# kalj/dealii-cuda

Hardware: AMD Instinct MI355X
Metric: DoFs/s on 1305x Laplace vmult (bmop), p=4 3D uniform (higher is better)
Workload: dtype f64; 1 GPU; bmop: DEGREE_FE=4, DIMENSION=3, MATRIX_FREE_UNIFORM_MESH, hyper_cube(-1,1), 54^3 cells, 10218313 DoFs, 1 z-slab(s); cells_per_dir=54, n_dofs=10218313, n_cells=157464, parallelism=slab1, dof_numbering=caller's (lexicographic), finite=True, clock_ramp_steps=2000

## Files before the change

### dealii-cuda_amd/csrc/mfgpu_kernels_p.hip

```cpp
#include <hip/hip_runtime.h>

#include "mfgpu_cell.h"
#include "mfgpu_kernels.h"
#include "mfgpu_planes.h"

namespace mfgpu {

#define MFGPU_PIN_VMEM() __builtin_amdgcn_sched_barrier(0x380)

template <int n, typename T, bool ADD, bool HN, bool SH = false, bool MASS = false>
__global__ void __launch_bounds__(64) __attribute__((amdgpu_waves_per_eu(1, 1)))
apply_planes3(const ApplyArgs<T> A, const TablesEO<T, n> tab) {
  constexpr int n2 = n * n;
  constexpr int CW = p_cells_per_wave(n);
  constexpr int NT = CW * n;
  constexpr int KGU = p_kgu(n);
  constexpr int JI = p_ji(n);
  constexpr int HS = KGU - JI;
  constexpr int SA = p_cell_stride(n);
  constexpr int NIW = (n2 + 1) / 2;
  extern __shared__ __attribute__((aligned(16))) unsigned char smem_raw[];
  constexpr int PRIV = HN ? p_priv_max(n) : 0;
  double *ua = reinterpret_cast<double *>(smem_raw);
  T *Aw = reinterpret_cast<T *>(ua + KGU * 64 + PRIV + (HN ? n2 : 0));
  T *Bw = Aw + (CW + 1) * SA;
  double *Wl = ua + KGU * 64 + PRIV;

  const int lane = threadIdx.x;
  if (HN) {
    if (lane < n2) Wl[lane] = (double)A.hn_weights[lane];
  }
  const int lc = lane / n, k = lane - lc * n;
  const bool lane_on = lane < NT;
  const int tk = lane_on ? lane : NT - 1;

  uint32_t b, bstride, bend;
  {
    const uint32_t nbt = A.batch_end - A.batch0 - A.hole_len, G = gridDim.x;
    if (G >= 8 && nbt >= G) {
      const uint32_t xcd = blockIdx.x & 7u, slot = blockIdx.x >> 3;
      const uint32_t q = G >> 3, rem = G & 7u;
      const uint32_t wlo = xcd * q + (xcd < rem ? xcd : rem);
      const uint32_t w = q + (xcd < rem ? 1u : 0u);
      b = A.batch0 + (uint32_t)((uint64_t)nbt * wlo / G) + slot;
      bend = A.batch0 + (uint32_t)((uint64_t)nbt * (wlo + w) / G);
      bstride = w;
    } else {
      b = A.batch0 + blockIdx.x;
      bend = A.batch_end - A.hole_len;
      bstride = G;
    }
  }
  if (b >= bend) return;
  const uint32_t hole0 = A.hole0, hole_len = A.hole_len;
  auto next_of = [&](uint32_t x) {
    const uint32_t l = (x >= hole0 ? x - hole_len : x) + bstride;
    return l < bend ? (l >= hole0 ? l + hole_len : l) : x;
  };
  if (b >= hole0) b += hole_len;
  static_assert(kernel_exists(PlaneKernel::planes3, n, number_type_of<T>, HN, SH, MASS), "no such instantiation");
  struct Meta {
    uint32_t base, drec, irec;
  };
  auto meta_request = [&](uint32_t bb) -> uint32_t {
    return A.shtab[(size_t)bb * kShBatchWords + (lane & (kShBatchWords - 1))];
  };
  auto meta_of = [&](uint32_t v) -> Meta {
    return Meta{(uint32_t)__builtin_amdgcn_readlane((int)v, 0), (uint32_t)__builtin_amdgcn_readlane((int)v, 1),
                (uint32_t)__builtin_amdgcn_readlane((int)v, 2)};
  };

  auto load_dofs = [&](uint32_t rec, uint32_t (&g)[KGU]) {
    const uint32_t *p = A.bdofsp + (size_t)rec * (KGU * 64) + lane;
#pragma unroll
    for (int j = 0; j < KGU; ++j) g[j] = SH ? p[j * 64] : nt_load(p + j * 64);
  };
  auto src_at = [&](uint32_t base, uint32_t g) -> T {
    const T *const sp = SH ? A.src + base : A.src;
    return *reinterpret_cast<const T *>(reinterpret_cast<const char *>(sp) + (uint32_t)(g * (uint32_t)sizeof(T)));
  };
  auto dst_at = [&](uint32_t base, uint32_t g) -> T * {
    T *const dp = SH ? A.dst + base : A.dst;
    return reinterpret_cast<T *>(reinterpret_cast<char *>(dp) + (uint32_t)(g * (uint32_t)sizeof(T)));
  };
  auto load_ix = [&](uint32_t rec, uint32_t (&ix)[NIW]) {
    const uint32_t *p = A.idxp + (size_t)rec * (NIW * NT) + tk;
#pragma unroll
    for (int w = 0; w < NIW; ++w) ix[w] = SH ? p[w * NT] : nt_load(p + w * NT);
  };
  auto stage_src = [&](const uint32_t (&g)[KGU], const T (&sv)[KGU]) {
#pragma unroll
    for (int j = 0; j < KGU; ++j) {
      double v = (double)sv[j];
      if (j >= JI) {
        const unsigned long long keep = (unsigned long long)(long long)~((int)g[j] >> 31);
        v = __longlong_as_double((long long)((unsigned long long)__double_as_longlong(v) & keep));
      }
      ua[lane + j * 64] = v;
    }
  };
  auto ixb = [&](const uint32_t (&ix)[NIW], int i) -> uint32_t {
    return (i & 1) ? (ix[i >> 1] >> 16) : (ix[i >> 1] & 0xffffu);
  };
  auto scatter_slot = [&](int j, uint32_t bb, uint32_t base, uint32_t g, T r, T oldv) {
    if (j < JI) {
      *dst_at(base, g) = ADD ? oldv + r : r;
    } else {
      T *const hp = A.halo + (size_t)bb * (HS * 64) + lane;
      hp[(j - JI) * 64] = r;
    }
  };

  uint32_t b1 = next_of(b), b2 = next_of(b1);
  uint32_t Gp[KGU], Gc[KGU], Gn[KGU], Gnn[KGU];
  uint32_t IXc[NIW], IXn[NIW];
  constexpr int CR = PRIV / 64, HROWS = HN ? p_hn_rows(n) : 1;
  uint32_t Hc[HROWS], Hn[HROWS];
  auto load_hn = [&](uint32_t bb, uint32_t (&H)[HROWS]) {
    const uint32_t slot = A.hn_slot[bb];
    if (slot != 0xffffffffu) {
      const uint32_t *p = A.hnrec + (size_t)slot * (HROWS * 64) + lane;
#pragma unroll
      for (int w = 0; w < HROWS; ++w) H[w] = nt_load(p + w * 64);
    } else {
#pragma unroll
      for (int w = 0; w < HROWS; ++w) H[w] = 0u;
    }
  };
  T Cc[n2];
  T Mm[MASS ? n2 : 1];
  T SVn[KGU], R[KGU], old[KGU];
  Meta Mp{0u, 0u, 0u}, Mc = Mp, M1 = Mp, M2 = Mp;
  uint32_t Mv = 0u;
  if (SH) {
    Mc = meta_of(meta_request(b));
    M1 = meta_of(meta_request(b1));
    M2 = meta_of(meta_request(b2));
    Mp = Mc;
  }
  load_dofs(SH ? Mc.drec : b, Gc);
  load_dofs(SH ? M1.drec : b1, Gn);
  load_ix(SH ? Mc.irec : b, IXc);
  if (HN) load_hn(b, Hc);
  constexpr uint32_t kDummyIx = 8u * (uint32_t)(KGU * 64 - 1) * 0x10001u;
#pragma unroll
  for (int w = 0; w < NIW; ++w) IXc[w] = lane_on ? IXc[w] : kDummyIx;
  {
    const T *p = A.coefp + (size_t)b * (n2 * NT) + tk;
#pragma unroll
    for (int r = 0; r < n2; ++r) Cc[r] = nt_load(p + r * NT);
  }
  if (MASS) {
    const T *p = A.massp + (size_t)b * (n2 * NT) + tk;
#pragma unroll
    for (int r = 0; r < n2; ++r) Mm[r] = nt_load(p + r * NT);
  }
#pragma unroll
  for (int j = 0; j < KGU; ++j) {
    SVn[j] = src_at(Mc.base, Gc[j]);
    Gp[j] = Gc[j];
    R[j] = T(0);
    old[j] = T(0);
  }
  stage_src(Gc, SVn);
  WaveSync::sync();

  const int pxy = lc * SA + n2 * k;
  const int pyz = lc * SA + k;
  uint32_t bp = b;

  while (true) {
    const bool has_next = b1 != b;
    constexpr int kH2 = HN ? HROWS - 2 : 0, kH1 = HN ? HROWS - 1 : 0;
    const uint32_t hn_ncopy = HN ? (uint32_t)__builtin_amdgcn_readfirstlane(Hc[kH2] & 0xffffu) : 0u;
    auto hn_count = [&](int dir) -> uint32_t {
      const uint32_t w = dir == 0 ? Hc[kH2] >> 16 : dir == 1 ? Hc[kH1] & 0xffffu : Hc[kH1] >> 16;
      return (uint32_t)__builtin_amdgcn_readfirstlane(w);
    };
    auto hn_pass = [&](int dir, bool transposed, const double (&Wr)[n2]) {
      const uint32_t count = hn_count(dir);
#pragma unroll
      for (int r = 0; r < kHnOpRounds; ++r) {
        if ((uint32_t)(r * 64) >= count) break;
        const bool on = (uint32_t)(r * 64 + lane) < count;
        const uint32_t *ww = &Hc[CR + (dir * kHnOpRounds + r) * 3];
        double v[n], o[n];
        uint32_t pos[n];
#pragma unroll
        for (int t = 0; t < n; ++t) {
          pos[t] = on ? (ww[t >> 1] >> (16 * (t & 1))) & 0xffffu : (uint32_t)(KGU * 64 + PRIV - 1);
          v[t] = ua[pos[t]];
        }
#pragma unroll
        for (int i = 0; i < n; ++i) {
          double acc = 0.0;
#pragma unroll
          for (int k2 = 0; k2 < n; ++k2) acc = fma(transposed ? Wr[k2 * n + i] : Wr[i * n + k2], v[k2], acc);
          o[i] = acc;
        }
        if (on) {
#pragma unroll
          for (int i = 0; i < n; ++i) ua[pos[i]] = o[i];
        }
      }
    };
    if (HN && hn_ncopy) {
      double Wr[n2];
#pragma unroll
      for (int i = 0; i < n2; ++i) Wr[i] = Wl[i];
      double cv[CR > 0 ? CR : 1];
#pragma unroll
      for (int r = 0; r < CR; ++r) cv[r] = (uint32_t)(r * 64 + lane) < hn_ncopy ? ua[Hc[r] & 0xffffu] : 0.0;
#pragma unroll
      for (int r = 0; r < CR; ++r)
        if ((uint32_t)(r * 64 + lane) < hn_ncopy) ua[Hc[r] >> 16] = cv[r];
      WaveSync::sync();
      hn_pass(0, false, Wr);
      WaveSync::sync();
      hn_pass(1, false, Wr);
      WaveSync::sync();
      hn_pass(2, false, Wr);
      WaveSync::sync();
    }
    STAMP(0);
    RSTAMP(8);
    WGSTAMP(10);
    load_dofs(SH ? M2.drec : b2, Gnn);
    load_ix(SH ? M1.irec : b1, IXn);
    if (SH) Mv = meta_request(next_of(b2));
    if (HN) load_hn(b1, Hn);
    if (ADD) {
#pragma unroll
      for (int j = 0; j < JI; ++j) old[j] = *dst_at(Mp.base, Gp[j]);
    }
    STAMP(1);
    auto hookA = [&](int) {};
    auto hookB = [&](int s) {
      MFGPU_PIN_VMEM();
#pragma unroll
      for (int j = (KGU * s) / (5 * n); j < (KGU * (s + 1)) / (5 * n); ++j)
        scatter_slot(j, bp, Mp.base, Gp[j], R[j], old[j]);
#pragma unroll
      for (int j = (KGU * s) / (5 * n); j < (KGU * (s + 1)) / (5 * n); ++j)
        SVn[j] = src_at(M1.base, Gn[j]);
      MFGPU_PIN_VMEM();
    };
    const T *const cnext = A.coefp + (size_t)b1 * (n2 * NT) + tk;
    const T *const mnext = MASS ? A.massp + (size_t)b1 * (n2 * NT) + tk : nullptr;
    auto hookC = [&](int s) {
      MFGPU_PIN_VMEM();
#pragma unroll
      for (int r = (n2 * s) / (2 * n); r < (n2 * (s + 1)) / (2 * n); ++r)
        Cc[r] = nt_load(cnext + r * NT);
      if (MASS) {
#pragma unroll
        for (int r = (n2 * s) / (2 * n); r < (n2 * (s + 1)) / (2 * n); ++r)
          Mm[r] = nt_load(mnext + r * NT);
      }
      MFGPU_PIN_VMEM();
    };

    {
      T u[n2];
#pragma unroll
      for (int x = 0; x < n; ++x)
#pragma unroll
        for (int y = 0; y < n; ++y)
          u[x + n * y] = (T) * reinterpret_cast<const double *>(reinterpret_cast<const char *>(ua) + ixb(IXc, x + n * y));
#pragma unroll
      for (int x = 0; x < n; ++x) {
        T in[n], out[n];
        get_line<n, 1>(u, x, in);
        eo_apply<n, 0>(tab, in, out);
        set_line<n, 1>(u, x, out);
        hookA(x);
      }
#pragma unroll
      for (int y = 0; y < n; ++y) {
        T in[n], a[n], bb[n];
        get_line<n, 0>(u, y, in);
        eo_apply<n, 0>(tab, in, a);
        eo_apply<n, 2>(tab, a, bb);
#pragma unroll
        for (int x = 0; x < n; ++x) {
          Aw[pxy + x + n * y] = a[x];
          Bw[pxy + x + n * y] = bb[x];
        }
        hookA(n + y);
      }
    }
    WaveSync::sync();
    STAMP(2);
#pragma unroll
    for (int j = 0; j < KGU + PRIV / 64; ++j) ua[lane + j * 64] = 0.0;

    {
      T nx[n];
#pragma unroll
      for (int z = 0; z < n; ++z) nx[z] = Bw[pyz + n2 * z];
#pragma unroll
      for (int y = 0; y < n; ++y) {
        T in[n], g[n], o[n];
#pragma unroll
        for (int z = 0; z < n; ++z) in[z] = nx[z];
#pragma unroll
        for (int z = 0; z < n; ++z) nx[z] = y + 1 < n ? Bw[pyz + n * (y + 1) + n2 * z] : Aw[pyz + n2 * z];
        eo_apply<n, 0>(tab, in, g);
#pragma unroll
        for (int z = 0; z < n; ++z) g[z] *= Cc[y + n * z];
        eo_apply<n, 1>(tab, g, o);
#pragma unroll
        for (int z = 0; z < n; ++z) Bw[pyz + n * y + n2 * z] = o[z];
        hookB(y);
      }
      T v[n2], r[n2];
#pragma unroll
      for (int y = 0; y < n; ++y) {
        T in[n], o[n];
#pragma unroll
        for (int z = 0; z < n; ++z) in[z] = nx[z];
        if (y + 1 < n) {
#pragma unroll
          for (int z = 0; z < n; ++z) nx[z] = Aw[pyz + n * (y + 1) + n2 * z];
        }
        eo_apply<n, 0>(tab, in, o);
        set_line<n, 1>(v, y, o);
        hookB(n + y);
      }
#pragma unroll
      for (int y = 0; y < n; ++y) {
        T in[n], g[n], o[n];
        get_line<n, 1>(v, y, in);
        eo_apply<n, 2>(tab, in, g);
#pragma unroll
        for (int z = 0; z < n; ++z) g[z] *= Cc[y + n * z];
        eo_apply<n, 3>(tab, g, o);
        set_line<n, 1>(r, y, o);
        hookB(2 * n + y);
      }
#pragma unroll
      for (int z = 0; z < n; ++z) {
        T in[n], g[n], o[n];
        get_line<n, 0>(v, z, in);
        eo_apply<n, 2>(tab, in, g);
#pragma unroll
        for (int y = 0; y < n; ++y) g[y] *= Cc[y + n * z];
        eo_apply<n, 3>(tab, g, o);
#pragma unroll
        for (int y = 0; y < n; ++y) r[y + n * z] += MASS ? fma(Mm[y + n * z], in[y], o[y]) : o[y];
        hookB(3 * n + z);
      }
#pragma unroll
      for (int y = 0; y < n; ++y) {
        T in[n], o[n];
        get_line<n, 1>(r, y, in);
        eo_apply<n, 1>(tab, in, o);
#pragma unroll
        for (int z = 0; z < n; ++z) Aw[pyz + n * y + n2 * z] = o[z];
        hookB(4 * n + y);
      }
    }
    WaveSync::sync();
    STAMP(3);

    {
      T o[n2];
      T nr[n], nt[n];
#pragma unroll
      for (int x = 0; x < n; ++x) {
        nr[x] = Aw[pxy + x];
        nt[x] = Bw[pxy + x];
      }
#pragma unroll
      for (int y = 0; y < n; ++y) {
        T rp[n], tp[n], w[n], ol[n];
#pragma unroll
        for (int x = 0; x < n; ++x) {
          rp[x] = nr[x];
          tp[x] = nt[x];
        }
        if (y + 1 < n) {
#pragma unroll
          for (int x = 0; x < n; ++x) {
            nr[x] = Aw[pxy + x + n * (y + 1)];
            nt[x] = Bw[pxy + x + n * (y + 1)];
          }
        }
        eo_apply<n, 3>(tab, tp, w);
#pragma unroll
        for (int x = 0; x < n; ++x) w[x] += rp[x];
        eo_apply<n, 1>(tab, w, ol);
        set_line<n, 0>(o, y, ol);
        hookC(y);
      }
#pragma unroll
      for (int x = 0; x < n; ++x) {
        T in[n], out[n];
        get_line<n, 1>(o, x, in);
        eo_apply<n, 1>(tab, in, out);
#pragma unroll
        for (int y = 0; y < n; ++y)
          lds_add(reinterpret_cast<double *>(reinterpret_cast<char *>(ua) + ixb(IXc, x + n * y)), (double)out[y]);
        hookC(n + x);
      }
    }
    WaveSync::sync();
    STAMP(4);

    if (HN && hn_ncopy) {
      double Wr[n2];
#pragma unroll
      for (int i = 0; i < n2; ++i) Wr[i] = Wl[i];
      hn_pass(2, true, Wr);
      WaveSync::sync();
      hn_pass(1, true, Wr);
      WaveSync::sync();
      hn_pass(0, true, Wr);
      WaveSync::sync();
      double cv[CR > 0 ? CR : 1];
#pragma unroll
      for (int r = 0; r < CR; ++r) cv[r] = (uint32_t)(r * 64 + lane) < hn_ncopy ? ua[Hc[r] >> 16] : 0.0;
#pragma unroll
      for (int r = 0; r < CR; ++r)
        if ((uint32_t)(r * 64 + lane) < hn_ncopy) lds_add(ua + (Hc[r] & 0xffffu), cv[r]);
      WaveSync::sync();
    }
#pragma unroll
    for (int j = 0; j < KGU; ++j) R[j] = (T)ua[lane + j * 64];
    WaveSync::sync();
    STAMP(5);
    stage_src(Gn, SVn);
    STAMP(6);
    bp = b;
    if (SH) Mp = Mc;
#pragma unroll
    for (int j = 0; j < KGU; ++j) Gp[j] = Gc[j];
    STAMP(7);
    RSTAMP(9);
    if (!has_next) break;
    WaveSync::sync();
    b = b1;
    b1 = b2;
    b2 = next_of(b2);
    if (SH) {
      Mc = M1;
      M1 = M2;
      M2 = meta_of(Mv);
    }
#pragma unroll
    for (int j = 0; j < KGU; ++j) {
      Gc[j] = Gn[j];
      Gn[j] = Gnn[j];
    }
#pragma unroll
    for (int w = 0; w < NIW; ++w) IXc[w] = lane_on ? IXn[w] : kDummyIx;
    if (HN) {
#pragma unroll
      for (int w = 0; w < HROWS; ++w) Hc[w] = Hn[w];
    }
  }
  if (ADD) {
#pragma unroll
    for (int j = 0; j < JI; ++j) old[j] = *dst_at(Mp.base, Gp[j]);
  }
#pragma unroll
  for (int j = 0; j < KGU; ++j) scatter_slot(j, bp, Mp.base, Gp[j], R[j], old[j]);
}

template <int n, typename T>
static size_t p_lds_bytes(bool hn) {
  return ((size_t)p_kgu(n) * 64 + (hn ? (size_t)p_priv_max(n) + n * n : 0)) * sizeof(double) +
         (size_t)2 * (p_cells_per_wave(n) + 1) * p_cell_stride(n) * sizeof(T);
}

template <typename T>
hipError_t p_bind(int, int n, bool hn, bool, bool sh, bool mass, uint32_t, CellKernel<T> *k) {
  return dispatch_instantiation(n, [&](auto N, auto HN, auto SH, auto MASS) {
    constexpr int n_ = N;
    if constexpr (kernel_exists(PlaneKernel::planes3, n_, number_type_of<T>, HN, SH, MASS))
      return bind_cell_kernel<T, 64, apply_planes3<n_, T, false, HN, SH, MASS>, apply_planes3<n_, T, true, HN, SH, MASS>,
                              make_tables_eo<T, n_>>(p_lds_bytes<n_, T>(HN), k);
    else
      return hipErrorInvalidValue;
  }, hn, sh, mass);
}
template hipError_t p_bind<double>(int, int, bool, bool, bool, bool, uint32_t, CellKernel<double> *);
template hipError_t p_bind<float>(int, int, bool, bool, bool, bool, uint32_t, CellKernel<float> *);

template <typename T>
__global__ void relayout_coef_kernel(T *out, const T *in, const uint32_t *cell_batch, const uint32_t *cell_pos,
                                     size_t total, int n) {
  const size_t i = (size_t)blockIdx.x * blockDim.x + threadIdx.x;
  if (i >= total) return;
  const int n2 = n * n, nd = n2 * n, NT = (64 / n) * n;
  const size_t cell = i / nd;
  const int q = (int)(i - cell * nd);
  const int x = q % n, r = q / n;
  out[((size_t)cell_batch[cell] * n2 + r) * NT + cell_pos[cell] * n + x] = in[i];
}

template <typename T>
hipError_t relayout_coef_launch(T *out, const T *in, const uint32_t *cell_batch, const uint32_t *cell_pos,
                                size_t total, int n, hipStream_t st) {
  if (total == 0) return hipSuccess;
  hipLaunchKernelGGL(relayout_coef_kernel<T>, dim3((unsigned)((total + 255) / 256)), dim3(256), 0, st, out, in,
                     cell_batch, cell_pos, total, n);
  return hipGetLastError();
}
template hipError_t relayout_coef_launch<double>(double *, const double *, const uint32_t *, const uint32_t *, size_t,
                                                 int, hipStream_t);
template hipError_t relayout_coef_launch<float>(float *, const float *, const uint32_t *, const uint32_t *, size_t, int,
                                                hipStream_t);

}
```

### dealii-cuda_amd/csrc/mfgpu_kernels_q.hip

```cpp
#include <hip/hip_runtime.h>

#include "mfgpu_cell.h"
#include "mfgpu_kernels.h"
#include "mfgpu_planes.h"

namespace mfgpu {

#define MFGPU_PIN_VMEM() __builtin_amdgcn_sched_barrier(0x380)

template <int n, typename T, bool ADD, bool HN, bool MASS = false>
__device__ __forceinline__ void planes4_body(const ApplyArgs<T> &A, const TablesEO<T, n> &tab) {
  constexpr int n2 = n * n;
  constexpr int CW = p_cells_per_wave(n);
  constexpr int NT = CW * n;
  constexpr int KGU = p_kgu(n);
  constexpr int JI = p_ji(n);
  constexpr int HS = KGU - JI;
  constexpr int SA = q_cell_stride(n);
  constexpr int ZS = q_plane_stride(n);
  constexpr int NIW = (n2 + 1) / 2;
  constexpr int PRIV = HN ? p_priv_max(n) : 0;
  constexpr int NUA = KGU * 64 + PRIV;
  extern __shared__ __attribute__((aligned(16))) unsigned char smem_raw[];
  double *ua = reinterpret_cast<double *>(smem_raw);
  T *Tw = reinterpret_cast<T *>(smem_raw);
  double *Wl = reinterpret_cast<double *>(smem_raw) + q_region_doubles<T>(n);

  const int lane = threadIdx.x;
  if (HN) {
    if (lane < n2) Wl[lane] = (double)A.hn_weights[lane];
  }
  const int lc = lane / n, k = lane - lc * n;
  const bool lane_on = lane < NT;
  const int tk = lane_on ? lane : NT - 1;

  uint32_t b, bstride, bend;
  {
    const uint32_t nbt = A.batch_end - A.batch0 - A.hole_len, G = gridDim.x;
    if (G >= 8 && nbt >= G) {
      const uint32_t xcd = blockIdx.x & 7u, slot = blockIdx.x >> 3;
      const uint32_t q = G >> 3, rem = G & 7u;
      const uint32_t wlo = xcd * q + (xcd < rem ? xcd : rem);
      const uint32_t w = q + (xcd < rem ? 1u : 0u);
      b = A.batch0 + (uint32_t)((uint64_t)nbt * wlo / G) + slot;
      bend = A.batch0 + (uint32_t)((uint64_t)nbt * (wlo + w) / G);
      bstride = w;
    } else {
      b = A.batch0 + blockIdx.x;
      bend = A.batch_end - A.hole_len;
      bstride = G;
    }
  }
  if (b >= bend) return;
  const uint32_t hole0 = A.hole0, hole_len = A.hole_len;
  auto next_of = [&](uint32_t x) {
    const uint32_t l = (x >= hole0 ? x - hole_len : x) + bstride;
    return l < bend ? (l >= hole0 ? l + hole_len : l) : x;
  };
  if (b >= hole0) b += hole_len;

  auto load_dofs = [&](uint32_t bb, uint32_t (&g)[KGU]) {
    const uint32_t *p = A.bdofsp + (size_t)bb * (KGU * 64) + lane;
#pragma unroll
    for (int j = 0; j < KGU; ++j) g[j] = nt_load(p + j * 64);
  };
  auto src_at = [&](uint32_t g) -> T {
    return *reinterpret_cast<const T *>(reinterpret_cast<const char *>(A.src) + (uint32_t)(g * (uint32_t)sizeof(T)));
  };
  auto dst_at = [&](uint32_t g) -> T * {
    return reinterpret_cast<T *>(reinterpret_cast<char *>(A.dst) + (uint32_t)(g * (uint32_t)sizeof(T)));
  };
  auto load_ix = [&](uint32_t bb, uint32_t (&ix)[NIW]) {
    const uint32_t *p = A.idxp + (size_t)bb * (NIW * NT) + tk;
#pragma unroll
    for (int w = 0; w < NIW; ++w) ix[w] = nt_load(p + w * NT);
  };
  auto load_coef = [&](uint32_t bb, T (&c)[n2]) {
    const T *p = A.coefp + (size_t)bb * (n2 * NT) + tk;
#pragma unroll
    for (int r = 0; r < n2; ++r) c[r] = nt_load(p + r * NT);
  };
  auto stage_src = [&](const uint32_t (&g)[KGU], const T (&sv)[KGU]) {
#pragma unroll
    for (int j = 0; j < KGU; ++j) {
      double v = (double)sv[j];
      if (j >= JI) {
        const unsigned long long keep = (unsigned long long)(long long)~((int)g[j] >> 31);
        v = __longlong_as_double((long long)((unsigned long long)__double_as_longlong(v) & keep));
      }
      ua[lane + j * 64] = v;
    }
  };
  auto ixb = [&](const uint32_t (&ix)[NIW], int i) -> uint32_t {
    return (i & 1) ? (ix[i >> 1] >> 16) : (ix[i >> 1] & 0xffffu);
  };
  constexpr uint32_t kDummyIx = 8u * (uint32_t)(KGU * 64 - 1) * 0x10001u;

  uint32_t b1 = next_of(b);
  uint32_t Gc[KGU], IXc[NIW];
  T Cc[n2], SV[KGU];
  constexpr int CR = PRIV / 64, HROWS = HN ? p_hn_rows(n) : 1;
  uint32_t Hc[HROWS];
  auto load_hn = [&](uint32_t bb, uint32_t (&H)[HROWS]) {
    const uint32_t slot = A.hn_slot[bb];
    if (slot != 0xffffffffu) {
      const uint32_t *p = A.hnrec + (size_t)slot * (HROWS * 64) + lane;
#pragma unroll
      for (int w = 0; w < HROWS; ++w) H[w] = nt_load(p + w * 64);
    } else {
#pragma unroll
      for (int w = 0; w < HROWS; ++w) H[w] = 0u;
    }
  };
  load_dofs(b, Gc);
  load_ix(b, IXc);
  if (HN) load_hn(b, Hc);
#pragma unroll
  for (int j = 0; j < KGU; ++j) SV[j] = src_at(Gc[j]);
  constexpr bool kCoefInS1 = n >= 6;
  if (!kCoefInS1) load_coef(b, Cc);
#pragma unroll
  for (int w = 0; w < NIW; ++w) IXc[w] = lane_on ? IXc[w] : kDummyIx;

  const int pxy = lc * SA + ZS * k;
  const int pyz = lc * SA + k;

  while (true) {
    const bool has_next = b1 != b;
    stage_src(Gc, SV);
    WaveSync::sync();

    constexpr int kH2 = HN ? HROWS - 2 : 0, kH1 = HN ? HROWS - 1 : 0;
    const uint32_t hn_ncopy = HN ? (uint32_t)__builtin_amdgcn_readfirstlane(Hc[kH2] & 0xffffu) : 0u;
    auto hn_count = [&](int dir) -> uint32_t {
      const uint32_t w = dir == 0 ? Hc[kH2] >> 16 : dir == 1 ? Hc[kH1] & 0xffffu : Hc[kH1] >> 16;
      return (uint32_t)__builtin_amdgcn_readfirstlane(w);
    };
    auto hn_pass = [&](int dir, bool transposed, const double (&Wr)[n2]) {
      const uint32_t count = hn_count(dir);
#pragma unroll
      for (int r = 0; r < kHnOpRounds; ++r) {
        if ((uint32_t)(r * 64) >= count) break;
        const bool on = (uint32_t)(r * 64 + lane) < count;
        const uint32_t *ww = &Hc[CR + (dir * kHnOpRounds + r) * 3];
        double v[n], o[n];
        uint32_t pos[n];
#pragma unroll
        for (int t = 0; t < n; ++t) {
          pos[t] = on ? (ww[t >> 1] >> (16 * (t & 1))) & 0xffffu : (uint32_t)(NUA - 1);
          v[t] = ua[pos[t]];
        }
#pragma unroll
        for (int i = 0; i < n; ++i) {
          double acc = 0.0;
#pragma unroll
          for (int k2 = 0; k2 < n; ++k2) acc = fma(transposed ? Wr[k2 * n + i] : Wr[i * n + k2], v[k2], acc);
          o[i] = acc;
        }
        if (on) {
#pragma unroll
          for (int i = 0; i < n; ++i) ua[pos[i]] = o[i];
        }
      }
    };
    if (HN && hn_ncopy) {
      double Wr[n2];
#pragma unroll
      for (int i = 0; i < n2; ++i) Wr[i] = Wl[i];
      double cv[CR > 0 ? CR : 1];
#pragma unroll
      for (int r = 0; r < CR; ++r) cv[r] = (uint32_t)(r * 64 + lane) < hn_ncopy ? ua[Hc[r] & 0xffffu] : 0.0;
#pragma unroll
      for (int r = 0; r < CR; ++r)
        if ((uint32_t)(r * 64 + lane) < hn_ncopy) ua[Hc[r] >> 16] = cv[r];
      WaveSync::sync();
      hn_pass(0, false, Wr);
      WaveSync::sync();
      hn_pass(1, false, Wr);
      WaveSync::sync();
      hn_pass(2, false, Wr);
      WaveSync::sync();
    }

    const T *const cthis = A.coefp + (size_t)b * (n2 * NT) + tk;
    auto hook_coef = [&](int s) {
      MFGPU_PIN_VMEM();
#pragma unroll
      for (int r = (n2 * s) / (2 * n); r < (n2 * (s + 1)) / (2 * n); ++r) Cc[r] = nt_load(cthis + r * NT);
      MFGPU_PIN_VMEM();
    };
    T u[n2];
#pragma unroll
    for (int i = 0; i < n2; ++i)
      u[i] = (T) * reinterpret_cast<const double *>(reinterpret_cast<const char *>(ua) + ixb(IXc, i));
    WaveSync::sync();
#pragma unroll
    for (int x = 0; x < n; ++x) {
      T in[n], out[n];
      get_line<n, 1>(u, x, in);
      eo_apply<n, 0>(tab, in, out);
      set_line<n, 1>(u, x, out);
      if (kCoefInS1) hook_coef(x);
    }
#pragma unroll
    for (int y = 0; y < n; ++y) {
      T in[n], a[n], bb[n];
      get_line<n, 0>(u, y, in);
      eo_apply<n, 0>(tab, in, a);
      eo_apply<n, 2>(tab, a, bb);
      set_line<n, 0>(u, y, a);
#pragma unroll
      for (int x = 0; x < n; ++x) Tw[pxy + x + n * y] = bb[x];
      if (kCoefInS1) hook_coef(n + y);
    }
    WaveSync::sync();

    constexpr bool kIxInS2 = n == 6;
    uint32_t IXn[NIW];
    const uint32_t *const ixnext = A.idxp + (size_t)b1 * (NIW * NT) + tk;
#pragma unroll
    for (int y = 0; y < n; ++y) {
      T in[n], g[n], o[n];
#pragma unroll
      for (int z = 0; z < n; ++z) in[z] = Tw[pyz + n * y + ZS * z];
      eo_apply<n, 0>(tab, in, g);
#pragma unroll
      for (int z = 0; z < n; ++z) g[z] *= Cc[y + n * z];
      eo_apply<n, 1>(tab, g, o);
#pragma unroll
      for (int z = 0; z < n; ++z) Tw[pyz + n * y + ZS * z] = o[z];
      if (kIxInS2) {
        MFGPU_PIN_VMEM();
#pragma unroll
        for (int i = (NIW * y) / n; i < (NIW * (y + 1)) / n; ++i) IXn[i] = nt_load(ixnext + i * NT);
        MFGPU_PIN_VMEM();
      }
    }
    WaveSync::sync();

    uint32_t Gn[KGU];
    load_dofs(b1, Gn);
    T Mm[MASS ? n2 : 1];
    const T *const mthis = MASS ? A.massp + (size_t)b * (n2 * NT) + tk : nullptr;

    T w[n2];
#pragma unroll
    for (int y = 0; y < n; ++y) {
      T tp[n], wl[n];
#pragma unroll
      for (int x = 0; x < n; ++x) tp[x] = Tw[pxy + x + n * y];
      eo_apply<n, 3>(tab, tp, wl);
      set_line<n, 0>(w, y, wl);
#pragma unroll
      for (int x = 0; x < n; ++x) Tw[pxy + x + n * y] = u[x + n * y];
      if (MASS) {
        MFGPU_PIN_VMEM();
#pragma unroll
        for (int r = n * y; r < n * (y + 1); ++r) Mm[r] = nt_load(mthis + r * NT);
        MFGPU_PIN_VMEM();
      }
    }
    WaveSync::sync();

    {
      T v[n2];
#pragma unroll
      for (int y = 0; y < n; ++y) {
        T in[n], o[n];
#pragma unroll
        for (int z = 0; z < n; ++z) in[z] = Tw[pyz + n * y + ZS * z];
        eo_apply<n, 0>(tab, in, o);
        set_line<n, 1>(v, y, o);
      }
#pragma unroll
      for (int y = 0; y < n; ++y) {
        T in[n], g[n], o[n], o2[n];
        get_line<n, 1>(v, y, in);
        eo_apply<n, 2>(tab, in, g);
#pragma unroll
        for (int z = 0; z < n; ++z) g[z] *= Cc[y + n * z];
        eo_apply<n, 3>(tab, g, o);
        eo_apply<n, 1>(tab, o, o2);
#pragma unroll
        for (int z = 0; z < n; ++z) Tw[pyz + n * y + ZS * z] = o2[z];
      }
#pragma unroll
      for (int z = 0; z < n; ++z) {
        T in[n], g[n], o[n];
        get_line<n, 0>(v, z, in);
        eo_apply<n, 2>(tab, in, g);
#pragma unroll
        for (int y = 0; y < n; ++y) g[y] *= Cc[y + n * z];
        eo_apply<n, 3>(tab, g, o);
        if (MASS) {
#pragma unroll
          for (int y = 0; y < n; ++y) o[y] = fma(Mm[y + n * z], in[y], o[y]);
        }
        set_line<n, 0>(v, z, o);
      }
#pragma unroll
      for (int y = 0; y < n; ++y) {
        T in[n], o[n];
        get_line<n, 1>(v, y, in);
        eo_apply<n, 1>(tab, in, o);
#pragma unroll
        for (int z = 0; z < n; ++z) lds_add(&Tw[pyz + n * y + ZS * z], o[z]);
      }
    }
    WaveSync::sync();

    uint32_t Hn[HROWS];
    if (HN) load_hn(b1, Hn);
    const T *const cnext = A.coefp + (size_t)b1 * (n2 * NT) + tk;
    auto hook = [&](int s) {
      constexpr int NIX = kIxInS2 ? 0 : NIW;
      constexpr int NL = KGU + NIX + (kCoefInS1 ? 0 : n2);
      MFGPU_PIN_VMEM();
#pragma unroll
      for (int i = (NL * s) / (2 * n); i < (NL * (s + 1)) / (2 * n); ++i) {
        if (i < KGU) SV[i] = src_at(Gn[i]);
        else if (i < KGU + NIX) IXn[i - KGU] = nt_load(ixnext + (i - KGU) * NT);
        else if (!kCoefInS1) Cc[i - KGU - NIX] = nt_load(cnext + (i - KGU - NIX) * NT);
      }
      MFGPU_PIN_VMEM();
    };

#pragma unroll
    for (int y = 0; y < n; ++y) {
      T rp[n], s2[n], ol[n];
#pragma unroll
      for (int x = 0; x < n; ++x) rp[x] = Tw[pxy + x + n * y];
#pragma unroll
      for (int x = 0; x < n; ++x) s2[x] = w[x + n * y] + rp[x];
      eo_apply<n, 1>(tab, s2, ol);
      set_line<n, 0>(w, y, ol);
      hook(y);
    }
    WaveSync::sync();
#pragma unroll
    for (int j = 0; j < (NUA + 63) / 64; ++j) ua[lane + j * 64] = 0.0;
#pragma unroll
    for (int x = 0; x < n; ++x) {
      T in[n], out[n];
      get_line<n, 1>(w, x, in);
      eo_apply<n, 1>(tab, in, out);
      set_line<n, 1>(w, x, out);
      hook(n + x);
    }
    WaveSync::sync();
#pragma unroll
    for (int i = 0; i < n2; ++i)
      lds_add(reinterpret_cast<double *>(reinterpret_cast<char *>(ua) + ixb(IXc, i)), (double)w[i]);
    WaveSync::sync();

    if (HN && hn_ncopy) {
      double Wr[n2];
#pragma unroll
      for (int i = 0; i < n2; ++i) Wr[i] = Wl[i];
      hn_pass(2, true, Wr);
      WaveSync::sync();
      hn_pass(1, true, Wr);
      WaveSync::sync();
      hn_pass(0, true, Wr);
      WaveSync::sync();
      double cv[CR > 0 ? CR : 1];
#pragma unroll
      for (int r = 0; r < CR; ++r) cv[r] = (uint32_t)(r * 64 + lane) < hn_ncopy ? ua[Hc[r] >> 16] : 0.0;
#pragma unroll
      for (int r = 0; r < CR; ++r)
        if ((uint32_t)(r * 64 + lane) < hn_ncopy) lds_add(ua + (Hc[r] & 0xffffu), cv[r]);
      WaveSync::sync();
    }

    {
      T *const hp = A.halo + (size_t)b * (HS * 64) + lane;
#pragma unroll
      for (int j = 0; j < KGU; ++j) {
        const T r = (T)ua[lane + j * 64];
        if (j < JI) {
          T *const p = dst_at(Gc[j]);
          *p = ADD ? *p + r : r;
        } else {
          hp[(j - JI) * 64] = r;
        }
      }
    }
    WaveSync::sync();
    if (!has_next) break;
    b = b1;
    b1 = next_of(b1);
#pragma unroll
    for (int j = 0; j < KGU; ++j) Gc[j] = Gn[j];
#pragma unroll
    for (int w2 = 0; w2 < NIW; ++w2) IXc[w2] = lane_on ? IXn[w2] : kDummyIx;
    if (HN) {
#pragma unroll
      for (int w2 = 0; w2 < HROWS; ++w2) Hc[w2] = Hn[w2];
    }
  }
}

template <int n, typename T, bool ADD, bool HN, bool MASS = false>
__global__ void __launch_bounds__(64) __attribute__((amdgpu_waves_per_eu(2, 2)))
apply_planes4(const ApplyArgs<T> A, const TablesEO<T, n> tab) {
  planes4_body<n, T, ADD, HN, MASS>(A, tab);
}
template <int n, typename T, bool ADD>
__global__ void __launch_bounds__(64) __attribute__((amdgpu_waves_per_eu(1, 1)))
apply_planes4w(const ApplyArgs<T> A, const TablesEO<T, n> tab) {
  planes4_body<n, T, ADD, false>(A, tab);
}

template <typename T>
hipError_t q_bind(int, int n, bool hn, bool, bool sh, bool mass, uint32_t, CellKernel<T> *k) {
  return dispatch_instantiation(n, [&](auto N, auto HN, auto SH, auto MASS) {
    constexpr int n_ = N;
    if constexpr (!kernel_exists(PlaneKernel::planes4, n_, number_type_of<T>, HN, SH, MASS))
      return hipErrorInvalidValue;
    else if constexpr (planes4_wide(n_))
      return bind_cell_kernel<T, 64, apply_planes4w<n_, T, false>, apply_planes4w<n_, T, true>, make_tables_eo<T, n_>>(
          q_lds_bytes<T>(n_, false), k);
    else
      return bind_cell_kernel<T, 64, apply_planes4<n_, T, false, HN, MASS>, apply_planes4<n_, T, true, HN, MASS>,
                              make_tables_eo<T, n_>>(q_lds_bytes<T>(n_, HN), k);
  }, hn, sh, mass);
}
template hipError_t q_bind<double>(int, int, bool, bool, bool, bool, uint32_t, CellKernel<double> *);
template hipError_t q_bind<float>(int, int, bool, bool, bool, bool, uint32_t, CellKernel<float> *);

}
```

### dealii-cuda_amd/csrc/mfgpu_planes.h

```cpp
#ifndef MFGPU_PLANES_H
#define MFGPU_PLANES_H

#include <hip/hip_runtime.h>

namespace mfgpu {

namespace {

template <typename U>
__device__ __forceinline__ U nt_load(const U *p) { return __builtin_nontemporal_load(p); }

template <int n, int DIR, typename T>
__device__ __forceinline__ void get_line(const T (&p)[n * n], int o, T (&l)[n]) {
#pragma unroll
  for (int i = 0; i < n; ++i) l[i] = p[DIR == 0 ? i + n * o : o + n * i];
}
template <int n, int DIR, typename T>
__device__ __forceinline__ void set_line(T (&p)[n * n], int o, const T (&l)[n]) {
#pragma unroll
  for (int i = 0; i < n; ++i) p[DIR == 0 ? i + n * o : o + n * i] = l[i];
}


template <typename T, int n>
struct TablesEO {
  static constexpr int h = n / 2, m = (n + 1) / 2;
  T Se[m * m], So[h * h], De[m * h], Do[h * m];
};

template <int n, int KIND, typename T>
__device__ __forceinline__ void eo_apply(const TablesEO<T, n> &tb, const T (&in)[n], T (&out)[n]) {
  constexpr int h = n / 2, m = (n + 1) / 2, p = n - 1;
  constexpr bool odd = (n & 1) != 0;
  T e[m], o[h > 0 ? h : 1];
#pragma unroll
  for (int k = 0; k < h; ++k) {
    e[k] = in[k] + in[p - k];
    o[k] = in[k] - in[p - k];
  }
  if (odd) e[h] = in[h];
  T E[m], O[h > 0 ? h : 1];
  if (KIND == 0 || KIND == 1) {
#pragma unroll
    for (int q = 0; q < m; ++q) {
      T t = (KIND == 0 ? tb.Se[0 * m + q] : tb.Se[q * m + 0]) * e[0];
#pragma unroll
      for (int k = 1; k < m; ++k) t = fma(KIND == 0 ? tb.Se[k * m + q] : tb.Se[q * m + k], e[k], t);
      E[q] = t;
    }
#pragma unroll
    for (int q = 0; q < h; ++q) {
      T t = (KIND == 0 ? tb.So[0 * h + q] : tb.So[q * h + 0]) * o[0];
#pragma unroll
      for (int k = 1; k < h; ++k) t = fma(KIND == 0 ? tb.So[k * h + q] : tb.So[q * h + k], o[k], t);
      O[q] = t;
    }
  } else if (KIND == 2) {
#pragma unroll
    for (int q = 0; q < m; ++q) {
      T t = tb.De[q * h + 0] * o[0];
#pragma unroll
      for (int k = 1; k < h; ++k) t = fma(tb.De[q * h + k], o[k], t);
      E[q] = t;
    }
#pragma unroll
    for (int q = 0; q < h; ++q) {
      T t = tb.Do[q * m + 0] * e[0];
#pragma unroll
      for (int k = 1; k < m; ++k) t = fma(tb.Do[q * m + k], e[k], t);
      O[q] = t;
    }
  } else {
#pragma unroll
    for (int q = 0; q < m; ++q) {
      T t = tb.Do[0 * m + q] * o[0];
#pragma unroll
      for (int k = 1; k < h; ++k) t = fma(tb.Do[k * m + q], o[k], t);
      E[q] = t;
    }
#pragma unroll
    for (int q = 0; q < h; ++q) {
      T t = tb.De[0 * h + q] * e[0];
#pragma unroll
      for (int k = 1; k < m; ++k) t = fma(tb.De[k * h + q], e[k], t);
      O[q] = t;
    }
  }
#pragma unroll
  for (int q = 0; q < h; ++q) {
    out[q] = E[q] + O[q];
    out[p - q] = E[q] - O[q];
  }
  if (odd) out[h] = E[h];
}


template <typename T, int n>
inline TablesEO<T, n> make_tables_eo(const double *S, const double *Dt) {
  TablesEO<T, n> tab;
  constexpr int h = n / 2, m = (n + 1) / 2, p = n - 1;
  for (int k = 0; k < m; ++k)
    for (int q = 0; q < m; ++q)
      tab.Se[k * m + q] = (T)((k < h && q < h) ? 0.5 * (S[k * n + q] + S[(p - k) * n + q]) : S[k * n + q]);
  for (int k = 0; k < h; ++k)
    for (int q = 0; q < h; ++q) tab.So[k * h + q] = (T)(0.5 * (S[k * n + q] - S[(p - k) * n + q]));
  for (int q = 0; q < m; ++q)
    for (int t = 0; t < h; ++t)
      tab.De[q * h + t] = (T)(q < h ? 0.5 * (Dt[q * n + t] - Dt[q * n + (p - t)]) : Dt[q * n + t]);
  for (int q = 0; q < h; ++q)
    for (int t = 0; t < m; ++t)
      tab.Do[q * m + t] = (T)(t < h ? 0.5 * (Dt[q * n + t] + Dt[q * n + (p - t)]) : Dt[q * n + t]);
  return tab;
}

}

}
#endif
```

Before: 79.12 billion DoFs/s.

## Chain even-odd sum-factorization stages in parity space, skipping join/split pairs

Splits eo_apply into split, products and join steps so consecutive 1D kernels can stay in even/odd parity form. The intermediate join-then-split between back-to-back applications is skipped, with a half-scaling of the middle term for odd n. Sums of two results are also accumulated directly in parity space, which removes redundant add/sub work and an lds_add read-modify-write in the q kernel. The trade-off is extra live parity registers (rz[n], wp[n]), which can add register pressure. The q kernel therefore disables this path for f64 with n=5 or 7.

```diff
diff --git a/dealii-cuda_amd/csrc/mfgpu_kernels_p.hip b/dealii-cuda_amd/csrc/mfgpu_kernels_p.hip
--- a/dealii-cuda_amd/csrc/mfgpu_kernels_p.hip
+++ b/dealii-cuda_amd/csrc/mfgpu_kernels_p.hip
@@ -279,8 +279,13 @@
       for (int y = 0; y < n; ++y) {
         T in[n], a[n], bb[n];
         get_line<n, 0>(u, y, in);
-        eo_apply<n, 0>(tab, in, a);
-        eo_apply<n, 2>(tab, a, bb);
+        Parity<T, n> s, ra, rb;
+        eo_split<n>(in, s);
+        eo_products<n, 0>(tab, s, ra);
+        eo_join<n>(ra, a);
+        eo_chain<n>(ra);
+        eo_products<n, 2>(tab, ra, rb);
+        eo_join<n>(rb, bb);
 #pragma unroll
         for (int x = 0; x < n; ++x) {
           Aw[pxy + x + n * y] = a[x];
@@ -314,28 +319,29 @@
         hookB(y);
       }
       T v[n2], r[n2];
+      Parity<T, n> rz[n];
 #pragma unroll
       for (int y = 0; y < n; ++y) {
-        T in[n], o[n];
+        T in[n], o[n], g[n];
 #pragma unroll
         for (int z = 0; z < n; ++z) in[z] = nx[z];
         if (y + 1 < n) {
 #pragma unroll
           for (int z = 0; z < n; ++z) nx[z] = Aw[pyz + n * (y + 1) + n2 * z];
         }
-        eo_apply<n, 0>(tab, in, o);
+        Parity<T, n> s, rv, rg;
+        eo_split<n>(in, s);
+        eo_products<n, 0>(tab, s, rv);
+        eo_join<n>(rv, o);
         set_line<n, 1>(v, y, o);
         hookB(n + y);
-      }
-#pragma unroll
-      for (int y = 0; y < n; ++y) {
-        T in[n], g[n], o[n];
-        get_line<n, 1>(v, y, in);
-        eo_apply<n, 2>(tab, in, g);
+        eo_chain<n>(rv);
+        eo_products<n, 2>(tab, rv, rg);
+        eo_join<n>(rg, g);
 #pragma unroll
         for (int z = 0; z < n; ++z) g[z] *= Cc[y + n * z];
-        eo_apply<n, 3>(tab, g, o);
-        set_line<n, 1>(r, y, o);
+        eo_split<n>(g, s);
+        eo_products<n, 3>(tab, s, rz[y]);
         hookB(2 * n + y);
       }
 #pragma unroll
@@ -347,14 +353,18 @@
         for (int y = 0; y < n; ++y) g[y] *= Cc[y + n * z];
         eo_apply<n, 3>(tab, g, o);
 #pragma unroll
-        for (int y = 0; y < n; ++y) r[y + n * z] += MASS ? fma(Mm[y + n * z], in[y], o[y]) : o[y];
+        for (int y = 0; y < n; ++y) r[y + n * z] = MASS ? fma(Mm[y + n * z], in[y], o[y]) : o[y];
         hookB(3 * n + z);
       }
 #pragma unroll
       for (int y = 0; y < n; ++y) {
         T in[n], o[n];
         get_line<n, 1>(r, y, in);
-        eo_apply<n, 1>(tab, in, o);
+        Parity<T, n> s, ro;
+        eo_split<n>(in, s);
+        eo_add<n>(rz[y], T(2), s);
+        eo_products<n, 1>(tab, s, ro);
+        eo_join<n>(ro, o);
 #pragma unroll
         for (int z = 0; z < n; ++z) Aw[pyz + n * y + n2 * z] = o[z];
         hookB(4 * n + y);
@@ -373,7 +383,7 @@
       }
 #pragma unroll
       for (int y = 0; y < n; ++y) {
-        T rp[n], tp[n], w[n], ol[n];
+        T rp[n], tp[n], ol[n];
 #pragma unroll
         for (int x = 0; x < n; ++x) {
           rp[x] = nr[x];
@@ -386,10 +396,13 @@
             nt[x] = Bw[pxy + x + n * (y + 1)];
           }
         }
-        eo_apply<n, 3>(tab, tp, w);
-#pragma unroll
-        for (int x = 0; x < n; ++x) w[x] += rp[x];
-        eo_apply<n, 1>(tab, w, ol);
+        Parity<T, n> s, rw, ro;
+        eo_split<n>(tp, s);
+        eo_products<n, 3>(tab, s, rw);
+        eo_split<n>(rp, s);
+        eo_add<n>(rw, T(2), s);
+        eo_products<n, 1>(tab, s, ro);
+        eo_join<n>(ro, ol);
         set_line<n, 0>(o, y, ol);
         hookC(y);
       }
diff --git a/dealii-cuda_amd/csrc/mfgpu_kernels_q.hip b/dealii-cuda_amd/csrc/mfgpu_kernels_q.hip
--- a/dealii-cuda_amd/csrc/mfgpu_kernels_q.hip
+++ b/dealii-cuda_amd/csrc/mfgpu_kernels_q.hip
@@ -21,6 +21,7 @@
   constexpr int NIW = (n2 + 1) / 2;
   constexpr int PRIV = HN ? p_priv_max(n) : 0;
   constexpr int NUA = KGU * 64 + PRIV;
+  constexpr bool kChained = !(sizeof(T) == 8 && (n == 5 || n == 7));
   extern __shared__ __attribute__((aligned(16))) unsigned char smem_raw[];
   double *ua = reinterpret_cast<double *>(smem_raw);
   T *Tw = reinterpret_cast<T *>(smem_raw);
@@ -206,8 +207,18 @@
     for (int y = 0; y < n; ++y) {
       T in[n], a[n], bb[n];
       get_line<n, 0>(u, y, in);
-      eo_apply<n, 0>(tab, in, a);
-      eo_apply<n, 2>(tab, a, bb);
+      if (kChained) {
+        Parity<T, n> s, ra, rb;
+        eo_split<n>(in, s);
+        eo_products<n, 0>(tab, s, ra);
+        eo_join<n>(ra, a);
+        eo_chain<n>(ra);
+        eo_products<n, 2>(tab, ra, rb);
+        eo_join<n>(rb, bb);
+      } else {
+        eo_apply<n, 0>(tab, in, a);
+        eo_apply<n, 2>(tab, a, bb);
+      }
       set_line<n, 0>(u, y, a);
 #pragma unroll
       for (int x = 0; x < n; ++x) Tw[pxy + x + n * y] = bb[x];
@@ -244,13 +255,20 @@
     const T *const mthis = MASS ? A.massp + (size_t)b * (n2 * NT) + tk : nullptr;
 
     T w[n2];
+    Parity<T, n> wp[n];
 #pragma unroll
     for (int y = 0; y < n; ++y) {
       T tp[n], wl[n];
 #pragma unroll
       for (int x = 0; x < n; ++x) tp[x] = Tw[pxy + x + n * y];
-      eo_apply<n, 3>(tab, tp, wl);
-      set_line<n, 0>(w, y, wl);
+      if (kChained) {
+        Parity<T, n> s;
+        eo_split<n>(tp, s);
+        eo_products<n, 3>(tab, s, wp[y]);
+      } else {
+        eo_apply<n, 3>(tab, tp, wl);
+        set_line<n, 0>(w, y, wl);
+      }
 #pragma unroll
       for (int x = 0; x < n; ++x) Tw[pxy + x + n * y] = u[x + n * y];
       if (MASS) {
@@ -264,25 +282,47 @@
 
     {
       T v[n2];
-#pragma unroll
-      for (int y = 0; y < n; ++y) {
-        T in[n], o[n];
-#pragma unroll
-        for (int z = 0; z < n; ++z) in[z] = Tw[pyz + n * y + ZS * z];
-        eo_apply<n, 0>(tab, in, o);
-        set_line<n, 1>(v, y, o);
-      }
-#pragma unroll
-      for (int y = 0; y < n; ++y) {
-        T in[n], g[n], o[n], o2[n];
-        get_line<n, 1>(v, y, in);
-        eo_apply<n, 2>(tab, in, g);
-#pragma unroll
-        for (int z = 0; z < n; ++z) g[z] *= Cc[y + n * z];
-        eo_apply<n, 3>(tab, g, o);
-        eo_apply<n, 1>(tab, o, o2);
-#pragma unroll
-        for (int z = 0; z < n; ++z) Tw[pyz + n * y + ZS * z] = o2[z];
+      Parity<T, n> rz[n];
+      if (kChained) {
+#pragma unroll
+        for (int y = 0; y < n; ++y) {
+          T in[n], g[n], o[n];
+#pragma unroll
+          for (int z = 0; z < n; ++z) in[z] = Tw[pyz + n * y + ZS * z];
+          Parity<T, n> s, rv, rg;
+          eo_split<n>(in, s);
+          eo_products<n, 0>(tab, s, rv);
+          eo_join<n>(rv, o);
+          set_line<n, 1>(v, y, o);
+          eo_chain<n>(rv);
+          eo_products<n, 2>(tab, rv, rg);
+          eo_join<n>(rg, g);
+#pragma unroll
+          for (int z = 0; z < n; ++z) g[z] *= Cc[y + n * z];
+          eo_split<n>(g, s);
+          eo_products<n, 3>(tab, s, rz[y]);
+        }
+      } else {
+#pragma unroll
+        for (int y = 0; y < n; ++y) {
+          T in[n], o[n];
+#pragma unroll
+          for (int z = 0; z < n; ++z) in[z] = Tw[pyz + n * y + ZS * z];
+          eo_apply<n, 0>(tab, in, o);
+          set_line<n, 1>(v, y, o);
+        }
+#pragma unroll
+        for (int y = 0; y < n; ++y) {
+          T in[n], g[n], o[n], o2[n];
+          get_line<n, 1>(v, y, in);
+          eo_apply<n, 2>(tab, in, g);
+#pragma unroll
+          for (int z = 0; z < n; ++z) g[z] *= Cc[y + n * z];
+          eo_apply<n, 3>(tab, g, o);
+          eo_apply<n, 1>(tab, o, o2);
+#pragma unroll
+          for (int z = 0; z < n; ++z) Tw[pyz + n * y + ZS * z] = o2[z];
+        }
       }
 #pragma unroll
       for (int z = 0; z < n; ++z) {
@@ -302,9 +342,19 @@
       for (int y = 0; y < n; ++y) {
         T in[n], o[n];
         get_line<n, 1>(v, y, in);
-        eo_apply<n, 1>(tab, in, o);
-#pragma unroll
-        for (int z = 0; z < n; ++z) lds_add(&Tw[pyz + n * y + ZS * z], o[z]);
+        if (kChained) {
+          Parity<T, n> s, ro;
+          eo_split<n>(in, s);
+          eo_add<n>(rz[y], T(2), s);
+          eo_products<n, 1>(tab, s, ro);
+          eo_join<n>(ro, o);
+#pragma unroll
+          for (int z = 0; z < n; ++z) Tw[pyz + n * y + ZS * z] = o[z];
+        } else {
+          eo_apply<n, 1>(tab, in, o);
+#pragma unroll
+          for (int z = 0; z < n; ++z) lds_add(&Tw[pyz + n * y + ZS * z], o[z]);
+        }
       }
     }
     WaveSync::sync();
@@ -330,9 +380,17 @@
       T rp[n], s2[n], ol[n];
 #pragma unroll
       for (int x = 0; x < n; ++x) rp[x] = Tw[pxy + x + n * y];
-#pragma unroll
-      for (int x = 0; x < n; ++x) s2[x] = w[x + n * y] + rp[x];
-      eo_apply<n, 1>(tab, s2, ol);
+      if (kChained) {
+        Parity<T, n> s, ro;
+        eo_split<n>(rp, s);
+        eo_add<n>(wp[y], T(2), s);
+        eo_products<n, 1>(tab, s, ro);
+        eo_join<n>(ro, ol);
+      } else {
+#pragma unroll
+        for (int x = 0; x < n; ++x) s2[x] = w[x + n * y] + rp[x];
+        eo_apply<n, 1>(tab, s2, ol);
+      }
       set_line<n, 0>(w, y, ol);
       hook(y);
     }
diff --git a/dealii-cuda_amd/csrc/mfgpu_planes.h b/dealii-cuda_amd/csrc/mfgpu_planes.h
--- a/dealii-cuda_amd/csrc/mfgpu_planes.h
+++ b/dealii-cuda_amd/csrc/mfgpu_planes.h
@@ -28,32 +28,53 @@
   T Se[m * m], So[h * h], De[m * h], Do[h * m];
 };
 
-template <int n, int KIND, typename T>
-__device__ __forceinline__ void eo_apply(const TablesEO<T, n> &tb, const T (&in)[n], T (&out)[n]) {
-  constexpr int h = n / 2, m = (n + 1) / 2, p = n - 1;
-  constexpr bool odd = (n & 1) != 0;
+template <typename T, int n>
+struct Parity {
+  static constexpr int h = n / 2, m = (n + 1) / 2;
   T e[m], o[h > 0 ? h : 1];
+};
+
+template <int n, typename T>
+__host__ __device__ __forceinline__ void eo_split(const T (&in)[n], Parity<T, n> &s) {
+  constexpr int h = n / 2, p = n - 1;
 #pragma unroll
   for (int k = 0; k < h; ++k) {
-    e[k] = in[k] + in[p - k];
-    o[k] = in[k] - in[p - k];
+    s.e[k] = in[k] + in[p - k];
+    s.o[k] = in[k] - in[p - k];
   }
-  if (odd) e[h] = in[h];
-  T E[m], O[h > 0 ? h : 1];
+  if (n & 1) s.e[h] = in[h];
+}
+
+template <int n, typename T>
+__host__ __device__ __forceinline__ void eo_join(const Parity<T, n> &r, T (&out)[n]) {
+  constexpr int h = n / 2, p = n - 1;
+#pragma unroll
+  for (int q = 0; q < h; ++q) {
+    out[q] = r.e[q] + r.o[q];
+    out[p - q] = r.e[q] - r.o[q];
+  }
+  if (n & 1) out[h] = r.e[h];
+}
+
+template <int n, int KIND, typename T>
+__host__ __device__ __forceinline__ void eo_products(const TablesEO<T, n> &tb, const Parity<T, n> &s, Parity<T, n> &r) {
+  constexpr int h = n / 2, m = (n + 1) / 2;
+  const T(&e)[m] = s.e;
+  const T(&o)[h > 0 ? h : 1] = s.o;
   if (KIND == 0 || KIND == 1) {
 #pragma unroll
     for (int q = 0; q < m; ++q) {
       T t = (KIND == 0 ? tb.Se[0 * m + q] : tb.Se[q * m + 0]) * e[0];
 #pragma unroll
       for (int k = 1; k < m; ++k) t = fma(KIND == 0 ? tb.Se[k * m + q] : tb.Se[q * m + k], e[k], t);
-      E[q] = t;
+      r.e[q] = t;
     }
 #pragma unroll
     for (int q = 0; q < h; ++q) {
       T t = (KIND == 0 ? tb.So[0 * h + q] : tb.So[q * h + 0]) * o[0];
 #pragma unroll
       for (int k = 1; k < h; ++k) t = fma(KIND == 0 ? tb.So[k * h + q] : tb.So[q * h + k], o[k], t);
-      O[q] = t;
+      r.o[q] = t;
     }
   } else if (KIND == 2) {
 #pragma unroll
@@ -61,14 +82,14 @@
       T t = tb.De[q * h + 0] * o[0];
 #pragma unroll
       for (int k = 1; k < h; ++k) t = fma(tb.De[q * h + k], o[k], t);
-      E[q] = t;
+      r.e[q] = t;
     }
 #pragma unroll
     for (int q = 0; q < h; ++q) {
       T t = tb.Do[q * m + 0] * e[0];
 #pragma unroll
       for (int k = 1; k < m; ++k) t = fma(tb.Do[q * m + k], e[k], t);
-      O[q] = t;
+      r.o[q] = t;
     }
   } else {
 #pragma unroll
@@ -76,22 +97,40 @@
       T t = tb.Do[0 * m + q] * o[0];
 #pragma unroll
       for (int k = 1; k < h; ++k) t = fma(tb.Do[k * m + q], o[k], t);
-      E[q] = t;
+      r.e[q] = t;
     }
 #pragma unroll
     for (int q = 0; q < h; ++q) {
       T t = tb.De[0 * h + q] * e[0];
 #pragma unroll
       for (int k = 1; k < m; ++k) t = fma(tb.De[k * h + q], e[k], t);
-      O[q] = t;
+      r.o[q] = t;
     }
   }
+}
+
+template <int n, typename T>
+__host__ __device__ __forceinline__ void eo_chain(Parity<T, n> &r) {
+  if (n & 1) r.e[n / 2] *= T(0.5);
+}
+
+template <int n, typename T>
+__host__ __device__ __forceinline__ void eo_add(const Parity<T, n> &r, T c, Parity<T, n> &s) {
+  constexpr int h = n / 2;
 #pragma unroll
-  for (int q = 0; q < h; ++q) {
-    out[q] = E[q] + O[q];
-    out[p - q] = E[q] - O[q];
+  for (int k = 0; k < h; ++k) {
+    s.e[k] = fma(r.e[k], T(2) * c, s.e[k]);
+    s.o[k] = fma(r.o[k], T(2) * c, s.o[k]);
   }
-  if (odd) out[h] = E[h];
+  if (n & 1) s.e[h] = fma(r.e[h], c, s.e[h]);
+}
+
+template <int n, int KIND, typename T>
+__host__ __device__ __forceinline__ void eo_apply(const TablesEO<T, n> &tb, const T (&in)[n], T (&out)[n]) {
+  Parity<T, n> s, r;
+  eo_split<n>(in, s);
+  eo_products<n, KIND>(tb, s, r);
+  eo_join<n>(r, out);
 }
 
 
```

Result: no change. 79.80 billion DoFs/s (median of 6 runs) (+0.9%).
